# jilljenn/TF-recomm

Measured on AMD Instinct MI355X. Metric: training ratings/sec + val RMSE, MovieLens-1M SVD dim=64 @1 GPU, higher is better.
Workload: dtype f32

## Files before the change

tf-recomm_amd/csrc/svd_kernels.hip:

```cpp
#include <hip/hip_runtime.h>
#include <stdint.h>
#include "svd_kernels.h"
#include "forward_body.h"
#include "finalize.inc.h"

namespace tfr {

template <int VEC>
__device__ __forceinline__ void store_frag(float* __restrict__ row, int d0, int D, const Frag<VEC>& f) {
    if (d0 < D) {
        if constexpr (VEC == 4) {
            *reinterpret_cast<float4*>(row + d0) = make_float4(f.v[0], f.v[1], f.v[2], f.v[3]);
        } else {
            row[d0] = f.v[0];
        }
    }
}

template <int VEC, bool NT>
__device__ __forceinline__ Frag<VEC> load_full(const float* __restrict__ p) {
    Frag<VEC> f;
    if constexpr (VEC == 4) {
        floatx4 t;
        if constexpr (NT) t = __builtin_nontemporal_load(reinterpret_cast<const floatx4*>(p));
        else t = *reinterpret_cast<const floatx4*>(p);
        f.v[0] = t.x; f.v[1] = t.y; f.v[2] = t.z; f.v[3] = t.w;
    } else {
        if constexpr (NT) f.v[0] = __builtin_nontemporal_load(p);
        else f.v[0] = *p;
    }
    return f;
}

template <int VEC>
__device__ __forceinline__ Frag<VEC> load_frag_h(const float* __restrict__ row, int d0, int D, bool nt) {
    return nt ? load_frag<VEC, true>(row, d0, D) : load_frag<VEC, false>(row, d0, D);
}
template <int VEC>
__device__ __forceinline__ void store_frag_h(float* __restrict__ row, int d0, int D, const Frag<VEC>& f, bool nt) {
    if (!nt) { store_frag<VEC>(row, d0, D, f); return; }
    if (d0 < D) {
        if constexpr (VEC == 4) {
            floatx4 t; t.x = f.v[0]; t.y = f.v[1]; t.z = f.v[2]; t.w = f.v[3];
            __builtin_nontemporal_store(t, reinterpret_cast<floatx4*>(row + d0));
        } else {
            __builtin_nontemporal_store(f.v[0], row + d0);
        }
    }
}

__device__ __forceinline__ __amdgpu_buffer_rsrc_t wt_rsrc(const void* base) {
    return __builtin_amdgcn_make_buffer_rsrc(const_cast<void*>(base), 0, 0x7fffffff, 0x00020000);
}
template <int VEC>
__device__ __forceinline__ void store_frag_wt(__amdgpu_buffer_rsrc_t r, size_t off, int d0, int D, const Frag<VEC>& f) {
    if (d0 < D) {
        if constexpr (VEC == 4) {
            typedef unsigned uintx4 __attribute__((ext_vector_type(4)));
            uintx4 t;
            t.x = __float_as_uint(f.v[0]); t.y = __float_as_uint(f.v[1]); t.z = __float_as_uint(f.v[2]); t.w = __float_as_uint(f.v[3]);
            __builtin_amdgcn_raw_buffer_store_b128(t, r, (int)((off + d0) * 4), 0, 16);
        } else {
            __builtin_amdgcn_raw_buffer_store_b32(__float_as_uint(f.v[0]), r, (int)((off + d0) * 4), 0, 16);
        }
    }
}
template <int VEC>
__device__ __forceinline__ void store_frag_p(float* base, size_t off, int d0, int D, const Frag<VEC>& f, bool wt) {
    if (wt) store_frag_wt<VEC>(wt_rsrc(base), off, d0, D, f);
    else store_frag<VEC>(base + off, d0, D, f);
}
__device__ __forceinline__ void store_word_p(void* base, size_t idx, uint32_t x, bool wt) {
    if (wt) __builtin_amdgcn_raw_buffer_store_b32(x, wt_rsrc(base), (int)(idx * 4), 0, 16);
    else reinterpret_cast<uint32_t*>(base)[idx] = x;
}

constexpr int BUF_NONE = (int)0x80000000u;
__device__ __forceinline__ uint32_t buf_load_word(__amdgpu_buffer_rsrc_t r, int byte_off) {
    return __builtin_amdgcn_raw_buffer_load_b32(r, byte_off, 0, 0);
}
template <int VEC>
__device__ __forceinline__ Frag<VEC> buf_load_frag(__amdgpu_buffer_rsrc_t r, int byte_off) {
    Frag<VEC> f;
    if constexpr (VEC == 4) {
        typedef unsigned uintx4 __attribute__((ext_vector_type(4)));
        const uintx4 t = __builtin_amdgcn_raw_buffer_load_b128(r, byte_off, 0, 0);
        f.v[0] = __uint_as_float(t.x); f.v[1] = __uint_as_float(t.y); f.v[2] = __uint_as_float(t.z); f.v[3] = __uint_as_float(t.w);
    } else {
        f.v[0] = __uint_as_float(buf_load_word(r, byte_off));
    }
    return f;
}

template <int G, int EPG>
__device__ __forceinline__ void block_sum_pieces(const float (&val)[3 * EPG], float* stage, float* out) {
    constexpr int EPB = 1024 / G;
    const int tid = threadIdx.x, lane = tid & 63, wave = tid >> 6;
    const int grp = tid / G, gl = tid % G;
    float* sl = stage;
    float* sg = stage + EPG * EPB;
    float* sr = stage + 2 * EPG * EPB;
#pragma unroll
    for (int h = 0; h < EPG; ++h) {
        if (gl == 0) { sl[h * EPB + grp] = val[3 * h + 0]; sg[h * EPB + grp] = val[3 * h + 2]; }
        sr[h * 1024 + tid] = val[3 * h + 1];
    }
    __syncthreads();
    if (wave < 3 * EPG) {
        const int h = wave / 3, c = wave % 3;
        float x = 0.f;
        if (c == 1) {
#pragma unroll
            for (int k = 0; k < 16; ++k) x += sr[h * 1024 + k * 64 + lane];
        } else {
            const float* src = (c == 0 ? sl : sg) + h * EPB;
            for (int k = lane; k < EPB; k += 64) x += src[k];
        }
        x = wave_sum(x);
        if (lane == 0) out[h * 4 + c] = x;
    }
}

template <int G, int VEC, int MODE, int UNR, bool PNT>
__global__ __launch_bounds__(256) void k_forward(FwdArgs a) {
    warm_args(a);
    forward_body<Float32Rows<VEC>, G, MODE, UNR, 4, PNT>(a, blockIdx.x, gridDim.x);
}
__device__ __forceinline__ void tile_scan_pack(int32_t* cnt, int nb, int32_t* wtot) {
    const int tid = threadIdx.x, lane = tid & 63, wave = tid >> 6;
    const int per = (nb + 1023) / 1024;
    int32_t sum = 0;
    for (int q = 0; q < per; ++q) { const int b = q * 1024 + tid; if (b < nb) sum += cnt[b]; }
    int32_t incl = sum;
#pragma unroll
    for (int o = 1; o < 64; o <<= 1) {
        const int32_t t2 = __shfl_up(incl, o, 64);
        if (lane >= o) incl += t2;
    }
    if (lane == 63) wtot[wave] = incl;
    __syncthreads();
    int32_t run = incl - sum;
    for (int w = 0; w < wave; ++w) run += wtot[w];
    for (int q = 0; q < per; ++q) {
        const int b = q * 1024 + tid;
        if (b < nb) { const int32_t c2 = cnt[b]; cnt[b] = (c2 << 16) | run; run += c2; }
    }
    __syncthreads();
}

template <int G, int VEC>
__global__ __launch_bounds__(1024) void k_front(FrontArgs fa) {
    warm_args(fa);
    if ((int)blockIdx.x < fa.nfwd) {
        forward_body<Float32Rows<VEC>, G, MODE_TRAIN, 2, 16>(fa.f, blockIdx.x, fa.nfwd);
        return;
    }
    extern __shared__ int32_t cnt[];
    const CSortArgs& a = fa.c;
    const int rb = blockIdx.x - fa.nfwd;
    const int col = rb / a.ntiles, tile = rb % a.ntiles, tid = threadIdx.x;
    const int nb = a.nbins[col];
    for (int b = tid; b < nb; b += CSORT_TILE) cnt[b] = 0;
    __syncthreads();
    const int64_t k = (int64_t)tile * CSORT_TILE + tid;
    const bool valid = k < a.B;
    int32_t key = 0, fullkey = 0;
    if (valid) {
        if (fa.f.ids) {
            int64_t id = fa.f.ids[k];
            if ((uint64_t)id >= (uint64_t)fa.f.N) id = 0;
            const int4 rec = fa.f.store[id];
            fullkey = col == 0 ? rec.x : rec.y;
            fa.key_out[col][k] = fullkey;
        } else {
            fullkey = a.keys[col][k];
        }
        key = fullkey & (nb - 1);
    }
    unsigned long long mask = __ballot(valid);
    for (int bit = 1; bit < nb; bit <<= 1) {
        const unsigned long long m = __ballot((key & bit) != 0);
        mask &= (key & bit) ? m : ~m;
    }
    const int lane = tid & 63, wave = tid >> 6;
    const unsigned long long below = mask & ((1ull << lane) - 1ull);
    const int rank_in_wave = __popcll(below);
    const int group_size = __popcll(mask);
    int base = 0;
    for (int w = 0; w < CSORT_TILE / 64; ++w) {
        if (wave == w && valid) {
            base = cnt[key];
            if (below == 0) cnt[key] = base + group_size;
        }
        __syncthreads();
    }
    if (!fa.tile_local) {
        if (valid) a.lrank[col][k] = base + rank_in_wave;
        for (int b = tid; b < nb; b += CSORT_TILE) a.hist[col][(size_t)tile * nb + b] = cnt[b];
        return;
    }
    __shared__ int32_t wtot[256];
    tile_scan_pack(cnt, nb, wtot);
    for (int b = tid; b < nb; b += CSORT_TILE) a.hist[col][(size_t)tile * nb + b] = cnt[b];
    if (valid) {
        const int64_t dst = (int64_t)tile * CSORT_TILE + (cnt[key] & 0xffff) + base + rank_in_wave;
        a.ks[col][dst] = fullkey;
        a.ps[col][dst] = (int32_t)k;
    }
}

struct TileLds {
    int32_t* cnt; int32_t* rec_u; int32_t* rec_i; float* rec_r; int32_t* srt_key; int32_t* srt_pos; int32_t* wtot;
};
__device__ __forceinline__ void tile_sort(int32_t* cnt_, int32_t* rec_u_, int32_t* rec_i_, float* rec_r_, int32_t* srt_key_,
                                          int32_t* srt_pos_, int32_t* wtot_, const int64_t* ids, const int4* store, const int4* recs,
                                          const int32_t* bu_, const int32_t* bi_, const float* br_, int64_t tile0, int nvalid, int side,
                                          int nb, int64_t N, int64_t U, int64_t I, int32_t* err, bool have_rec, int4 rec_in) {
    TileLds L;
    L.cnt = cnt_; L.rec_u = rec_u_; L.rec_i = rec_i_; L.rec_r = rec_r_; L.srt_key = srt_key_; L.srt_pos = srt_pos_; L.wtot = wtot_;
    const int tid = threadIdx.x, lane = tid & 63, wave = tid >> 6;
    for (int b = tid; b < nb; b += 1024) L.cnt[b] = 0;
    const bool valid = tid < nvalid;
    int32_t u = 0, it = 0;
    float r = 0.f;
    if (valid) {
        const int64_t k = tile0 + tid;
        bool oob = false;
        if (have_rec) {
            u = rec_in.x; it = rec_in.y; r = __int_as_float(rec_in.z);
        } else if (recs) {
            const int4 rec = recs[k];
            u = rec.x; it = rec.y; r = __int_as_float(rec.z);
        } else if (ids) {
            int64_t id = ids[k];
            if ((uint64_t)id >= (uint64_t)N) { atomicOr(err, 2); id = 0; }
            const int4 rec = store[id];
            u = rec.x; it = rec.y; r = __int_as_float(rec.z);
        } else {
            u = bu_[k]; it = bi_[k]; r = br_[k];
        }
        if ((uint64_t)(int64_t)u >= (uint64_t)U) { oob = true; u = 0; }
        if ((uint64_t)(int64_t)it >= (uint64_t)I) { oob = true; it = 0; }
        if (oob) atomicOr(err, 1);
    }
    L.rec_u[tid] = u; L.rec_i[tid] = it; L.rec_r[tid] = r;
    __syncthreads();
    const int32_t key = side == 0 ? u : it;
    unsigned long long mask = __ballot(valid);
    for (int bit = 1; bit < nb; bit <<= 1) {
        const unsigned long long mm = __ballot((key & bit) != 0);
        mask &= (key & bit) ? mm : ~mm;
    }
    const unsigned long long below = mask & ((1ull << lane) - 1ull);
    const int rank_in_wave = __popcll(below);
    const int group_size = __popcll(mask);
    int base = 0;
    for (int w = 0; w < 16; ++w) {
        if (wave == w && valid) {
            base = L.cnt[key];
            if (below == 0) L.cnt[key] = base + group_size;
        }
        __syncthreads();
    }
    tile_scan_pack(L.cnt, nb, L.wtot);
    if (valid) {
        const int dst = (L.cnt[key] & 0xffff) + base + rank_in_wave;
        L.srt_key[dst] = key;
        L.srt_pos[dst] = tid;
    }
    __syncthreads();
}

__device__ __forceinline__ void zero_tail(float* partials, int from, int to) {
    if (from < to) for (int k = from + (int)threadIdx.x; k < to; k += 1024) partials[k] = 0.f;
}

struct TileStamp {
    unsigned long long* p; unsigned long long t0;
    __device__ __forceinline__ void arm(unsigned long long* dbg) { p = dbg ? dbg + 8 * (size_t)blockIdx.x : nullptr; }
    __device__ __forceinline__ void mark(int k) const { if (p && threadIdx.x == 0) p[k] = __builtin_amdgcn_s_memrealtime(); }
    __device__ __forceinline__ ~TileStamp() { if (p && threadIdx.x == 0) { p[0] = t0; p[1] = __builtin_amdgcn_s_memrealtime(); } }
};

template <int G, int VEC, int EPG, bool PRE>
__device__ __forceinline__ void tile_pieces(const TileStepArgs& a, int32_t* dyn, const int32_t* rec_u, const int32_t* rec_i,
                                            const float* rec_r, const int32_t* srt_key, const int32_t* srt_pos, float* lds_gb,
                                            int32_t* lds_key, float* lds_stage, TileStamp& stamp, int side, int bx, int slice,
                                            int64_t tile0, int nvalid, const int4* srt, const WarmLines<TileStepArgs>& warm,
                                            int zero_from, int zero_to);

template <int G, int VEC, int EPG>
__global__ __launch_bounds__(1024) void k_tile_step(const int4* srt_u, const int4* srt_i, const int4* next_recs, int B, int nsort, int nblk_u,
                                                    int epg_item, int ntiles, int next_ntiles, int next_B, int stamps, TileStepArgs a) {
    const WarmLines<TileStepArgs> warm = warm_args_issue(a);
    constexpr int EPB = 1024 / G;
    extern __shared__ __attribute__((aligned(16))) int32_t dyn[];
    __shared__ int32_t rec_u[1024], rec_i[1024], srt_key[1024], srt_pos[1024];
    __shared__ float rec_r[1024];
    __shared__ __attribute__((aligned(16))) float lds_gb[2 * EPG * 16];
    __shared__ __attribute__((aligned(16))) int32_t lds_key[EPG * 16];
    __shared__ float lds_stage[EPG * (2 * EPB + 1024)];
    __shared__ int32_t wtot[16];
    static_assert(sizeof(rec_u) + sizeof(rec_i) + sizeof(srt_key) + sizeof(srt_pos) + sizeof(rec_r) + sizeof(lds_gb) + sizeof(lds_key) +
                  sizeof(lds_stage) + sizeof(wtot) == tile_step_static_lds(G, EPG), "tile_step_static_lds() is out of date");
    static_assert(tile_step_static_lds(G, EPG) + 64 * 1024 <= LDS_PER_CU, "static LDS leaves no room for 16384 sort bins");
    TileStamp stamp = {nullptr, stamps ? __builtin_amdgcn_s_memrealtime() : 0ull};
    const int tid = threadIdx.x;
    const bool ahead = (int)blockIdx.x < nsort;
    const int b0 = (int)blockIdx.x - nsort;
    const int side = ahead ? (int)blockIdx.x / next_ntiles : (b0 < nblk_u ? 0 : 1);
    const int bx = ahead ? 0 : (side ? b0 - nblk_u : b0);
    const int epg = side ? epg_item : EPG;
    const int EPS = EPB * epg;
    const int NSL = 1024 / EPS;
    const int tile = ahead ? (int)blockIdx.x % next_ntiles : bx / NSL;
    const int slice = bx % NSL;
    const int64_t tile0 = (int64_t)tile * 1024;
    const int Bt = ahead ? next_B : B;
    const int nvalid = (Bt - (int)tile0 < 1024) ? Bt - (int)tile0 : 1024;
    const int zero_from = (!ahead && side == 1 && (int64_t)(bx + 1) * EPS >= B) ? (bx + 1) * epg * 4 : INT32_MAX;
    const int zero_to = ntiles * G * 4;
    if (!ahead && slice * EPS >= nvalid) {
        stamp.arm(a.dbg);
        zero_tail(a.partials, zero_from, zero_to);
        if (side == 1 && tid < 4 * epg) a.partials[(size_t)bx * epg * 4 + tid] = 0.f;
        return;
    }
    if (!ahead && srt_u != nullptr) {
        const int4* srt = side ? srt_i : srt_u;
        if constexpr (EPG > 1) {
            if (epg != EPG) {
                tile_pieces<G, VEC, EPG / 2, true>(a, dyn, rec_u, rec_i, rec_r, srt_key, srt_pos, lds_gb, lds_key, lds_stage, stamp, side, bx,
                                                   slice, tile0, nvalid, srt, warm, zero_from, zero_to);
                return;
            }
        }
        tile_pieces<G, VEC, EPG, true>(a, dyn, rec_u, rec_i, rec_r, srt_key, srt_pos, lds_gb, lds_key, lds_stage, stamp, side, bx, slice,
                                       tile0, nvalid, srt, warm, zero_from, zero_to);
        return;
    }
    {
        const bool early = ahead && next_recs != nullptr;
        int4 early_rec = make_int4(0, 0, 0, 0);
        if (early) early_rec = next_recs[tile0 + (tid < nvalid ? tid : 0)];
        __builtin_amdgcn_sched_barrier(0);
        warm_args_land(warm);
        stamp.arm(a.dbg);
        zero_tail(a.partials, zero_from, zero_to);
        const int nb = a.nbins[side];
        tile_sort(dyn, rec_u, rec_i, rec_r, srt_key, srt_pos, wtot, ahead ? a.next_ids : a.ids, a.store, ahead ? next_recs : a.recs,
                  a.u, a.it, a.r, tile0, nvalid, side, nb, a.N, a.U, a.I, a.err, early, early_rec);
        const bool wt = a.wt & TFR_WT_PUBLISH;
        if (ahead) {
            int32_t* nt = a.next_tab[side];
            for (int b = tid; b < nb; b += 1024) store_word_p(nt, (size_t)tile * nb + b, (uint32_t)dyn[b], wt);
            if (tid < nvalid) {
                const int pl = srt_pos[tid];
                const int4 rec = make_int4(rec_u[pl], rec_i[pl], __float_as_int(rec_r[pl]), pl);
                if (wt) {
                    typedef unsigned uintx4 __attribute__((ext_vector_type(4)));
                    uintx4 t; t.x = (unsigned)rec.x; t.y = (unsigned)rec.y; t.z = (unsigned)rec.z; t.w = (unsigned)rec.w;
                    __builtin_amdgcn_raw_buffer_store_b128(t, wt_rsrc(a.next_srt[side]), (int)((tile0 + tid) * 16), 0, 16);
                } else {
                    a.next_srt[side][tile0 + tid] = rec;
                }
            }
            return;
        }
        const int nact = (nvalid + EPS - 1) / EPS;
        for (int b = slice * 1024 + tid; b < nb; b += nact * 1024) store_word_p(a.tab[side], (size_t)tile * nb + b, (uint32_t)dyn[b], wt);
        __syncthreads();
    }
    if constexpr (EPG > 1) {
        if (epg != EPG) {
            tile_pieces<G, VEC, EPG / 2, false>(a, dyn, rec_u, rec_i, rec_r, srt_key, srt_pos, lds_gb, lds_key, lds_stage, stamp, side, bx, slice,
                                                tile0, nvalid, nullptr, warm, zero_from, zero_to);
            return;
        }
    }
    tile_pieces<G, VEC, EPG, false>(a, dyn, rec_u, rec_i, rec_r, srt_key, srt_pos, lds_gb, lds_key, lds_stage, stamp, side, bx, slice, tile0,
                                    nvalid, nullptr, warm, zero_from, zero_to);
}

template <int G, int VEC, int EPG, bool PRE>
__device__ __forceinline__ void tile_pieces(const TileStepArgs& a, int32_t* dyn, const int32_t* rec_u, const int32_t* rec_i,
                                            const float* rec_r, const int32_t* srt_key, const int32_t* srt_pos, float* lds_gb,
                                            int32_t* lds_key, float* lds_stage, TileStamp& stamp, int side, int bx, int slice,
                                            int64_t tile0, int nvalid, const int4* srt, const WarmLines<TileStepArgs>& warm,
                                            int zero_from, int zero_to) {
    constexpr bool presorted = PRE;
    constexpr int EPB = 1024 / G;
    constexpr int EPS = EPB * EPG;
    const int tid = threadIdx.x;
    const int grp = tid / G, gl = tid % G, d0 = gl * VEC;
    int jl[EPG], bpos[EPG];
// ... 569 lines not shown
        if (gl == 0) {
            a.grad_bias[j] = gb;
            if (head && a.map) a.map[row] = (int32_t)j + 1;
        }
    } else if constexpr (RMODE == RMODE_ADAM) {
        if (!a.frozen_rows) {
            Frag<VEC> w;
            if constexpr (OWN_LDS) w = wre;
            else w = (FWD && LEAN) ? load_frag<VEC>(wsrc, d0, D) : o;
#pragma unroll
            for (int q = 0; q < VEC; ++q) adam_sparse(w.v[q], mrow.v[q], vrow.v[q], acc.v[q], c);
            const bool nts = FAST || (a.nt & 4);
            store_frag_h<VEC>(wdst, d0, D, w, nts);
            if (a.sel && gl == 0) a.sel[row] = cur ^ 1;
            store_frag_h<VEC>(a.m + roff, d0, D, mrow, nts);
            store_frag_h<VEC>(a.v + roff, d0, D, vrow, nts);
        }
        if (gl == 0 && !a.frozen_bias) {
            float w = ob;
            adam_sparse(w, mb, vb, gb, c);
            a.bias_w[row] = w;
            a.bias_m[row] = mb;
            a.bias_v[row] = vb;
        }
    } else if constexpr (RMODE == RMODE_SGD) {
        if (!a.frozen_rows) {
            Frag<VEC> w = o;
#pragma unroll
            for (int q = 0; q < VEC; ++q) w.v[q] = w.v[q] - a.lr * acc.v[q];
            store_frag<VEC>(wdst, d0, D, w);
            if (a.sel && gl == 0) a.sel[row] = cur ^ 1;
        }
        if (gl == 0 && !a.frozen_bias) a.bias_w[row] = ob - a.lr * gb;
    }
}

template <int VEC, int N>
__device__ __forceinline__ bool add_pieces(Frag<VEC>& t, float& gb, const float* __restrict__ grad_rows,
                                           const float* __restrict__ grad_bias, const int32_t* __restrict__ ks,
                                           int64_t B, int64_t safe, int64_t p, int64_t step, int32_t row, int d0, int D) {
    int32_t key[N];
#pragma unroll
    for (int q = 0; q < N; ++q) {
        const int64_t pp = p + (int64_t)q * step;
        key[q] = ks[pp < B ? pp : safe];
    }
    Frag<VEC> x[N];
    float xb[N];
#pragma unroll
    for (int q = 0; q < N; ++q) {
        const int64_t pp = (p + (int64_t)q * step < B) ? p + (int64_t)q * step : safe;
        x[q] = load_frag<VEC>(grad_rows + (size_t)pp * D, d0, D);
        xb[q] = grad_bias[pp];
    }
    bool go = true;
#pragma unroll
    for (int q = 0; q < N; ++q) {
        go = go && (p + (int64_t)q * step < B) && key[q] == row;
        if (go) {
#pragma unroll
            for (int e = 0; e < VEC; ++e) t.v[e] += x[q].v[e];
            gb += xb[q];
        }
    }
    return go;
}

template <int VEC, int PIECE>
__device__ __forceinline__ Frag<VEC> run_total(const float* __restrict__ grad_rows,
                                               const float* __restrict__ grad_bias,
                                               const int32_t* __restrict__ ks, int64_t B, int64_t j,
                                               int32_t row, int d0, int D, float& gb) {
    Frag<VEC> t = load_frag<VEC>(grad_rows + (size_t)j * D, d0, D);
    gb = grad_bias[j];
    int64_t p = (j / PIECE + 1) * PIECE;
    if (p >= B || ks[p] != row) return t;
    while (add_pieces<VEC, 8>(t, gb, grad_rows, grad_bias, ks, B, j, p, PIECE, row, d0, D)) p += 8 * (int64_t)PIECE;
    return t;
}

template <int G, int VEC, int OPT>
__global__ __launch_bounds__(256) void k_apply_rows(ApplyPair pr) {
    warm_args(pr.a[blockIdx.y]);
    constexpr int PIECE = 1024 / G;
    constexpr int GPB = 256 / G;
    constexpr int CW = 16;
    if (pr.with_fin && blockIdx.x == gridDim.x - 1) {
        if (blockIdx.y == 0) finalize_body(pr.f);
        return;
    }
    __shared__ float s_part[256 * VEC];
    __shared__ float s_partb[GPB];
    __shared__ long long s_next[GPB];
    __shared__ int32_t s_row[GPB];
    const ApplyArgs& a = pr.a[blockIdx.y];
    const int32_t err = *a.err;
    const int gl = threadIdx.x % G, grp = threadIdx.x / G;
    const int d0 = gl * VEC;
    const int D = a.D;
    const int64_t Bn = a.dB ? (int64_t)*a.dB : a.B;
    int64_t j = (int64_t)blockIdx.x * GPB + grp;
    int32_t row = 0;
    bool own;
    if (a.only_split) {
        const int64_t p = (j + 1) * PIECE;
        own = !err && p < Bn;
        if (own) {
            row = a.ks[p];
            const int64_t lo = p - PIECE;
            own = a.ks[p - 1] == row && !(lo > 0 && a.ks[lo - 1] == row);
            if (own) {
                const int sh = ((threadIdx.x % 64) / G) * G;
                j = p - 1;
                for (int k = 0; k < PIECE; k += G) {
                    const bool hit = (k + gl < PIECE) && a.ks[lo + k + gl] == row;
                    unsigned long long bits = __ballot(hit) >> sh;
                    if constexpr (G < 64) bits &= (1ull << G) - 1ull;
                    if (bits) { j = lo + k + (__ffsll((long long)bits) - 1); break; }
                }
            }
        }
    } else {
        own = !err && j < Bn;
        if (own) {
            row = a.ks[j];
            own = ((j > 0) ? a.ks[j - 1] : -2) != row;
        }
    }
    const size_t roff = (size_t)row * D;
    Frag<VEC> w, mrow, vrow, gr;
#pragma unroll
    for (int q = 0; q < VEC; ++q) { w.v[q] = 0.f; mrow.v[q] = 0.f; vrow.v[q] = 0.f; gr.v[q] = 0.f; }
    float gb = 0.f;
    long long next = -1;
    float* wtab = a.w;
    if (own) {
        if (a.sel && a.sel[row]) wtab = a.w_alt;
        if (OPT != 2 && !a.frozen_rows) {
            w = load_frag<VEC>(wtab + roff, d0, D);
            if constexpr (OPT == 0) {
                mrow = load_frag<VEC>(a.m + roff, d0, D);
                vrow = load_frag<VEC>(a.v + roff, d0, D);
            }
        }
        gr = load_frag<VEC>(a.grad_rows + (size_t)j * D, d0, D);
        gb = a.grad_bias[j];
        const int64_t p = (j / PIECE + 1) * PIECE;
        if (p < Bn && a.ks[p] == row &&
            add_pieces<VEC, 8>(gr, gb, a.grad_rows, a.grad_bias, a.ks, Bn, j, p, PIECE, row, d0, D))
            next = p + 8 * (int64_t)PIECE;
    }
    if (gl == 0) { s_next[grp] = next; s_row[grp] = row; }
    if (__syncthreads_or(next >= 0)) {
        for (int sl = 0; sl < GPB; ++sl) {
            const long long ps = s_next[sl];
            if (ps < 0) continue;
            const int32_t rs = s_row[sl];
            Frag<VEC> part;
#pragma unroll
            for (int q = 0; q < VEC; ++q) part.v[q] = 0.f;
            float pb = 0.f;
            int64_t pp = ps + (int64_t)grp * PIECE;
            while (add_pieces<VEC, CW>(part, pb, a.grad_rows, a.grad_bias, a.ks, Bn, 0, pp, (int64_t)GPB * PIECE, rs, d0, D))
                pp += (int64_t)CW * GPB * PIECE;
#pragma unroll
            for (int q = 0; q < VEC; ++q) s_part[threadIdx.x * VEC + q] = part.v[q];
            if (gl == 0) s_partb[grp] = pb;
            __syncthreads();
            if (grp == sl) {
                for (int g2 = 0; g2 < GPB; ++g2) {
#pragma unroll
                    for (int q = 0; q < VEC; ++q) gr.v[q] += s_part[(g2 * G + gl) * VEC + q];
                    gb += s_partb[g2];
                }
            }
            __syncthreads();
        }
    }
    if (!own) return;
    const AdamC c = {a.alpha, a.b1, a.b2, a.eps, 1.f - a.b1, 1.f - a.b2};
    if constexpr (OPT == 2) {
        store_frag<VEC>(a.w + (a.wstride ? (size_t)row * a.wstride : roff), d0, D, gr);
        if (gl == 0) a.bias_w[a.wbstride ? (size_t)row * a.wbstride : (size_t)row] = gb;
        return;
    }
    if (!a.frozen_rows) {
        if constexpr (OPT == 0) {
#pragma unroll
            for (int q = 0; q < VEC; ++q) adam_sparse(w.v[q], mrow.v[q], vrow.v[q], gr.v[q], c);
            store_frag<VEC>(a.m + roff, d0, D, mrow);
            store_frag<VEC>(a.v + roff, d0, D, vrow);
        } else {
#pragma unroll
            for (int q = 0; q < VEC; ++q) w.v[q] = w.v[q] - a.lr * gr.v[q];
        }
        store_frag<VEC>(wtab + roff, d0, D, w);
    }
    if (gl == 0 && !a.frozen_bias) {
        float bw = a.bias_w[row];
        if constexpr (OPT == 0) {
            float mb = a.bias_m[row], vb = a.bias_v[row];
            adam_sparse(bw, mb, vb, gb, c);
            a.bias_m[row] = mb;
            a.bias_v[row] = vb;
        } else {
            bw = bw - a.lr * gb;
        }
        a.bias_w[row] = bw;
    }
}

template <int G, int VEC>
__global__ __launch_bounds__(256) void k_adam_dense(DensePair pr) {
    constexpr int PIECE = 1024 / G;
    if (blockIdx.y == 2) {
        if (blockIdx.x == 0) finalize_body(pr.f);
        return;
    }
    warm_args(pr.a[blockIdx.y]);
    const DenseArgs& a = pr.a[blockIdx.y];
    if (*a.err) return;
    constexpr int GPB = 256 / G;
    const int gl = threadIdx.x % G;
    const int d0 = gl * VEC;
    const int D = a.D;
    const AdamC c = {a.alpha, a.b1, a.b2, a.eps, 1.f - a.b1, 1.f - a.b2};
    for (int64_t row = (int64_t)blockIdx.x * GPB + threadIdx.x / G; row < a.rows;
         row += (int64_t)gridDim.x * GPB) {
        const int32_t slot = a.map ? a.map[row] : 0;
        const size_t roff = (size_t)row * D;
        Frag<VEC> w, mrow, vrow;
#pragma unroll
        for (int q = 0; q < VEC; ++q) { w.v[q] = 0.f; mrow.v[q] = 0.f; vrow.v[q] = 0.f; }
        if (!a.frozen_rows) {
            w = load_frag<VEC>(a.w + roff, d0, D);
            if (a.opt == 0) {
                mrow = load_frag<VEC>(a.m + roff, d0, D);
                vrow = load_frag<VEC>(a.v + roff, d0, D);
            }
        }
        float bw = 0.f, mb = 0.f, vb = 0.f;
        if (gl == 0 && !a.frozen_bias) {
            bw = a.bias_w[row];
            if (a.opt == 0) { mb = a.bias_m[row]; vb = a.bias_v[row]; }
        }
        Frag<VEC> gr;
        float gb = 0.f;
        if (a.dense_grad) {
            gr = load_frag<VEC>(a.dense_grad + roff, d0, D);
            gb = a.dense_gbias[row];
            if (slot) {
                gr = run_total<VEC, PIECE>(a.grad_rows, a.grad_bias, a.ks, a.B, (int64_t)slot - 1, (int32_t)row, d0, D, gb);
                if (gl == 0) a.map[row] = 0;
            }
            Frag<VEC> z;
#pragma unroll
            for (int q = 0; q < VEC; ++q) z.v[q] = 0.f;
            store_frag<VEC>(a.dense_grad + roff, d0, D, z);
            if (gl == 0) a.dense_gbias[row] = 0.f;
        } else if (slot) {
            gr = run_total<VEC, PIECE>(a.grad_rows, a.grad_bias, a.ks, a.B, (int64_t)slot - 1, (int32_t)row, d0, D, gb);
            if (gl == 0) a.map[row] = 0;
        } else {
#pragma unroll
            for (int q = 0; q < VEC; ++q) gr.v[q] = 0.f;
        }
        if (!a.frozen_rows) {
            if (a.opt == 0) {
#pragma unroll
                for (int q = 0; q < VEC; ++q) adam_sparse(w.v[q], mrow.v[q], vrow.v[q], gr.v[q], c);
                store_frag<VEC>(a.m + roff, d0, D, mrow);
                store_frag<VEC>(a.v + roff, d0, D, vrow);
            } else {
#pragma unroll
                for (int q = 0; q < VEC; ++q) w.v[q] = w.v[q] - a.lr * gr.v[q];
            }
            store_frag<VEC>(a.w + roff, d0, D, w);
        }
        if (gl == 0 && !a.frozen_bias) {
            if (a.opt == 0) {
                adam_sparse(bw, mb, vb, gb, c);
                a.bias_m[row] = mb;
                a.bias_v[row] = vb;
            } else {
                bw = bw - a.lr * gb;
            }
            a.bias_w[row] = bw;
        }
    }
}

struct DenseHead { const int32_t* tab; const int32_t* err; int nbins, rows, ntiles; };
template <int G, int VEC, bool WRITE, int NT>
__device__ __forceinline__ void dense_tiles_rounds(const TileDenseLaunch& L, const DenseHead& h, const WarmLines<TileDenseArgs>& warm) {
    const TileDenseArgs& a = L.a[blockIdx.y];
    constexpr int GPB = 256 / G;
    constexpr int EPB = 1024 / G;
    constexpr int D = G * VEC;
    constexpr int NB = (NT > 12) ? 8 : NT;
    const int gl = threadIdx.x % G;
    const int d0 = gl * VEC;
    const int row = (int)blockIdx.x * GPB + threadIdx.x / G;
    if (row >= h.rows) return;
    const __amdgpu_buffer_rsrc_t rtab =
        __builtin_amdgcn_make_buffer_rsrc(const_cast<int32_t*>(h.tab), 0, h.ntiles * h.nbins * 4, 0x00020000);
    int32_t ent[NT];
#pragma unroll
    for (int t = 0; t < NT; ++t) ent[t] = (int32_t)buf_load_word(rtab, (t * h.nbins + row) * 4);
    int32_t err = (int32_t)buf_load_word(wt_rsrc(h.err), 0);
    __builtin_amdgcn_sched_barrier(0);
    warm_args_land(warm);
    const int roff = (row * D + d0) * 4;
    Frag<VEC> w, mrow, vrow;
    float bw = 0.f, mb = 0.f, vb = 0.f;
    if constexpr (!WRITE) {
        const int ow = a.frozen_rows ? BUF_NONE : roff;
        const int om = (a.frozen_rows || a.opt != 0) ? BUF_NONE : roff;
        w = buf_load_frag<VEC>(wt_rsrc(a.w), ow);
        mrow = buf_load_frag<VEC>(wt_rsrc(a.m), om);
        vrow = buf_load_frag<VEC>(wt_rsrc(a.v), om);
        const int ob = (gl == 0 && !a.frozen_bias) ? row * 4 : BUF_NONE;
        const int obm = (gl == 0 && !a.frozen_bias && a.opt == 0) ? row * 4 : BUF_NONE;
        bw = __uint_as_float(buf_load_word(wt_rsrc(a.bias_w), ob));
        mb = __uint_as_float(buf_load_word(wt_rsrc(a.bias_m), obm));
        vb = __uint_as_float(buf_load_word(wt_rsrc(a.bias_v), obm));
    }
    __builtin_amdgcn_sched_barrier(0);
    asm volatile("" : "+v"(err) : : "memory");
    if (err) return;
    int s0 = -1, s1 = -1, nk1 = 0;
    bool deep = false, touched = false;
#pragma unroll
    for (int t = 0; t < NT; ++t) {
        const int32_t e = ent[t];
        const int off = e & 0xffff;
        const int pp = t * 1024 + (off / EPB + 1) * EPB;
        const int end = t * 1024 + off + (e >> 16);
        const bool has1 = pp < end;
        deep = deep || pp + EPB < end;
        s1 = (has1 && nk1 == 1) ? pp : s1;
        s0 = (has1 && nk1 == 0) ? pp : s0;
        nk1 += has1 ? 1 : 0;
        touched = touched || (e >> 16);
    }
    const __amdgpu_buffer_rsrc_t rg = wt_rsrc(a.grad_rows), rgb = wt_rsrc(a.grad_bias);
    Frag<VEC> tot, c0, c1;
#pragma unroll
    for (int q = 0; q < VEC; ++q) tot.v[q] = 0.f;
    float gb = 0.f, cb0 = 0.f, cb1 = 0.f;
#pragma unroll
    for (int t0 = 0; t0 < NT; t0 += NB) {
        Frag<VEC> x[NB];
        float xb[NB];
#pragma unroll
        for (int t = 0; t < NB; ++t) {
            const int32_t e = ent[t0 + t];
            const int j = (t0 + t) * 1024 + (e & 0xffff);
            x[t] = buf_load_frag<VEC>(rg, (e >> 16) ? (j * D + d0) * 4 : BUF_NONE);
            xb[t] = __uint_as_float(buf_load_word(rgb, ((e >> 16) && gl == 0) ? j * 4 : BUF_NONE));
        }
        if (t0 == 0) {
            c0 = buf_load_frag<VEC>(rg, s0 >= 0 ? (s0 * D + d0) * 4 : BUF_NONE);
            cb0 = __uint_as_float(buf_load_word(rgb, (s0 >= 0 && gl == 0) ? s0 * 4 : BUF_NONE));
            c1 = buf_load_frag<VEC>(rg, s1 >= 0 ? (s1 * D + d0) * 4 : BUF_NONE);
            cb1 = __uint_as_float(buf_load_word(rgb, (s1 >= 0 && gl == 0) ? s1 * 4 : BUF_NONE));
        }
        __builtin_amdgcn_sched_barrier(0);
#pragma unroll
        for (int t = 0; t < NB; ++t) {
#pragma unroll
            for (int q = 0; q < VEC; ++q) tot.v[q] += x[t].v[q];
            gb += xb[t];
        }
    }
    if (nk1 <= 2 && !deep) {
#pragma unroll
        for (int q = 0; q < VEC; ++q) tot.v[q] += c0.v[q];
        gb += cb0;
#pragma unroll
        for (int q = 0; q < VEC; ++q) tot.v[q] += c1.v[q];
        gb += cb1;
    } else {
        for (int k = 1;; ++k) {
            bool more = false;
#pragma unroll
            for (int t0 = 0; t0 < NT; t0 += NB) {
                Frag<VEC> y[NB];
                float yb[NB];
#pragma unroll
                for (int t = 0; t < NB; ++t) {
                    const int32_t e = ent[t0 + t];
                    const int j = (t0 + t) * 1024 + (e & 0xffff);
                    const int pp = (j / EPB + k) * EPB;
                    const bool has = pp < j + (e >> 16);
                    y[t] = buf_load_frag<VEC>(rg, has ? (pp * D + d0) * 4 : BUF_NONE);
                    yb[t] = __uint_as_float(buf_load_word(rgb, (has && gl == 0) ? pp * 4 : BUF_NONE));
                    more = more || has;
                }
#pragma unroll
                for (int t = 0; t < NB; ++t) {
#pragma unroll
                    for (int q = 0; q < VEC; ++q) tot.v[q] += y[t].v[q];
                    gb += yb[t];
                }
            }
            if (!more) break;
        }
    }
    const size_t rfl = (size_t)row * D;
    if constexpr (WRITE) {
        if (touched) {
            store_frag<VEC>(a.out_rows + rfl, d0, D, tot);
            if (gl == 0) a.out_bias[row] = gb;
        }
    } else {
        if (!touched && a.skip_untouched) return;
        const AdamC c = {a.alpha, a.b1, a.b2, a.eps, 1.f - a.b1, 1.f - a.b2};
        const int wt = L.wt;
        if (!a.frozen_rows) {
            if (a.opt == 0) {
#pragma unroll
                for (int q = 0; q < VEC; ++q) adam_sparse(w.v[q], mrow.v[q], vrow.v[q], tot.v[q], c);
                store_frag_p<VEC>(a.m, rfl, d0, D, mrow, wt & TFR_WT_MOMENTS);
                store_frag_p<VEC>(a.v, rfl, d0, D, vrow, wt & TFR_WT_MOMENTS);
            } else {
#pragma unroll
                for (int q = 0; q < VEC; ++q) w.v[q] = __builtin_fmaf(-a.lr, tot.v[q], w.v[q]);
            }
            store_frag_p<VEC>(a.w, rfl, d0, D, w, wt & TFR_WT_ROWS);
        }
        if (gl == 0 && !a.frozen_bias) {
            const bool wb = wt & TFR_WT_BIAS;
            if (a.opt == 0) {
                adam_sparse(bw, mb, vb, gb, c);
                store_word_p(a.bias_m, (size_t)row, __float_as_uint(mb), wb);
                store_word_p(a.bias_v, (size_t)row, __float_as_uint(vb), wb);
            } else {
                bw = bw - __fmul_rn(a.lr, gb);
            }
            store_word_p(a.bias_w, (size_t)row, __float_as_uint(bw), wb);
        }
    }
}

template <int G, int VEC, bool WRITE, int NT>
__global__ __launch_bounds__(256, (NT > 12 && VEC == 4 && !WRITE) ? 2 : 3)
void k_dense_tiles(const int32_t* tab0, const int32_t* tab1, const int32_t* errp, int nbins0, int nbins1, int rows0, int rows1, int ntiles,
                   int ncols, int flags, TileDenseLaunch L) {
    const WarmLines<TileDenseArgs> warm = warm_args_issue(L.a[blockIdx.y]);
    if ((int)blockIdx.x == ncols) {
        if (blockIdx.y == 0 && (flags & DENSE_FLAG_FIN)) finalize_body(L.f);
        return;
    }
    const bool users = blockIdx.y != 0;
    const DenseHead h = {users ? tab1 : tab0, errp, users ? nbins1 : nbins0, users ? rows1 : rows0, ntiles};
    if constexpr (VEC == 4) {
        if (flags & DENSE_FLAG_ROUNDS) {
            dense_tiles_rounds<G, VEC, WRITE, NT>(L, h, warm);
            return;
        }
    }
    const TileDenseArgs& a = L.a[blockIdx.y];
    const int32_t err = *h.err;
    warm_args_land(warm);
    constexpr int GPB = 256 / G;
    constexpr int EPB = 1024 / G;
    const int gl = threadIdx.x % G;
    const int d0 = gl * VEC;
    const int D = a.D;
    const AdamC c = {a.alpha, a.b1, a.b2, a.eps, 1.f - a.b1, 1.f - a.b2};
    for (int64_t row = (int64_t)blockIdx.x * GPB + threadIdx.x / G; row < h.rows;
         row += (int64_t)ncols * GPB) {
        const size_t roff = (size_t)row * D;
        Frag<VEC> w, mrow, vrow;
#pragma unroll
        for (int q = 0; q < VEC; ++q) { w.v[q] = 0.f; mrow.v[q] = 0.f; vrow.v[q] = 0.f; }
        float bw = 0.f, mb = 0.f, vb = 0.f;
        if constexpr (!WRITE) {
            if (!a.frozen_rows) {
                w = load_frag<VEC>(a.w + roff, d0, D);
                if (a.opt == 0) {
                    mrow = load_frag<VEC>(a.m + roff, d0, D);
                    vrow = load_frag<VEC>(a.v + roff, d0, D);
                }
            }
            if (gl == 0 && !a.frozen_bias) {
                bw = a.bias_w[row];
                if (a.opt == 0) { mb = a.bias_m[row]; vb = a.bias_v[row]; }
            }
        }
        Frag<VEC> tot;
#pragma unroll
        for (int q = 0; q < VEC; ++q) tot.v[q] = 0.f;
        float gb = 0.f;
        bool touched = false;
        constexpr int NB = (NT > 12) ? 8 : NT;
        int32_t ent[NT];
#pragma unroll
        for (int t = 0; t < NT; ++t) ent[t] = (t < h.ntiles) ? h.tab[(size_t)t * h.nbins + row] : 0;
        if (err) return;
#pragma unroll
        for (int t0 = 0; t0 < NT; t0 += NB) {
            Frag<VEC> x[NB];
            float xb[NB];
#pragma unroll
            for (int t = 0; t < NB; ++t) {
                const int32_t e = ent[t0 + t];
#pragma unroll
                for (int q = 0; q < VEC; ++q) x[t].v[q] = 0.f;
                xb[t] = 0.f;
                if (e >> 16) {
                    const int64_t j = (int64_t)(t0 + t) * 1024 + (e & 0xffff);
                    x[t] = load_frag<VEC>(a.grad_rows + (size_t)j * D, d0, D);
                    xb[t] = a.grad_bias[j];
                }
            }
#pragma unroll
            for (int t = 0; t < NB; ++t) {
                if (ent[t0 + t] >> 16) {
                    touched = true;
#pragma unroll
                    for (int q = 0; q < VEC; ++q) tot.v[q] += x[t].v[q];
                    gb += xb[t];
                }
            }
        }
        for (int k = 1;; ++k) {
            bool more = false;
#pragma unroll
            for (int t0 = 0; t0 < NT; t0 += NB) {
                Frag<VEC> y[NB];
                float yb[NB];
#pragma unroll
                for (int t = 0; t < NB; ++t) {
                    const int32_t e = ent[t0 + t];
                    const int64_t j = (int64_t)(t0 + t) * 1024 + (e & 0xffff);
                    const int64_t pp = (j / EPB + k) * EPB;
                    const bool has = (e >> 16) && pp < j + (e >> 16);
#pragma unroll
                    for (int q = 0; q < VEC; ++q) y[t].v[q] = 0.f;
                    yb[t] = 0.f;
                    if (has) {
                        y[t] = load_frag<VEC>(a.grad_rows + (size_t)pp * D, d0, D);
                        yb[t] = a.grad_bias[pp];
                        more = true;
                    }
                }
#pragma unroll
                for (int t = 0; t < NB; ++t) {
#pragma unroll
                    for (int q = 0; q < VEC; ++q) tot.v[q] += y[t].v[q];
                    gb += yb[t];
                }
            }
            if (!more) break;
        }
        if constexpr (WRITE) {
            if (touched) {
                store_frag<VEC>(a.out_rows + roff, d0, D, tot);
                if (gl == 0) a.out_bias[row] = gb;
            }
        } else {
            if (!touched && a.skip_untouched) continue;
            const int wt = L.wt;
            if (!a.frozen_rows) {
                if (a.opt == 0) {
#pragma unroll
                    for (int q = 0; q < VEC; ++q) adam_sparse(w.v[q], mrow.v[q], vrow.v[q], tot.v[q], c);
                    store_frag_p<VEC>(a.m, roff, d0, D, mrow, wt & TFR_WT_MOMENTS);
                    store_frag_p<VEC>(a.v, roff, d0, D, vrow, wt & TFR_WT_MOMENTS);
                } else {
#pragma unroll
                    for (int q = 0; q < VEC; ++q) w.v[q] = w.v[q] - a.lr * tot.v[q];
                }
                store_frag_p<VEC>(a.w, roff, d0, D, w, wt & TFR_WT_ROWS);
            }
            if (gl == 0 && !a.frozen_bias) {
                const bool wb = wt & TFR_WT_BIAS;
                if (a.opt == 0) {
                    adam_sparse(bw, mb, vb, gb, c);
                    store_word_p(a.bias_m, (size_t)row, __float_as_uint(mb), wb);
                    store_word_p(a.bias_v, (size_t)row, __float_as_uint(vb), wb);
                } else {
                    bw = bw - a.lr * gb;
                }
                store_word_p(a.bias_w, (size_t)row, __float_as_uint(bw), wb);
            }
        }
    }
}

__global__ __launch_bounds__(256) void k_finalize(FinArgs a) { warm_args(a); finalize_body(a); }

__global__ __launch_bounds__(256) void k_auc_keys(const float* __restrict__ score, int32_t* __restrict__ keys, int64_t n) {
    for (int64_t k = (int64_t)blockIdx.x * blockDim.x + threadIdx.x; k < n; k += (int64_t)gridDim.x * blockDim.x) {
        float x = score[k];
        if (x == 0.f) x = 0.f;
        const uint32_t b = __float_as_uint(x);
        keys[k] = (int32_t)((b & 0x80000000u) ? ~b : (b | 0x80000000u));
    }
}

__global__ __launch_bounds__(256) void k_auc_ranksum(const int32_t* __restrict__ ks, const int32_t* __restrict__ ps,
                                                     const float* __restrict__ label, int64_t n, unsigned long long* out ) {
    unsigned long long s2 = 0, np = 0;
    for (int64_t j = (int64_t)blockIdx.x * blockDim.x + threadIdx.x; j < n; j += (int64_t)gridDim.x * blockDim.x) {
        if (label[ps[j]] > 0.5f) {
            const uint32_t key = (uint32_t)ks[j];
            int64_t lo = 0, hi = n;
            while (lo < hi) { const int64_t mid = (lo + hi) >> 1; if ((uint32_t)ks[mid] < key) lo = mid + 1; else hi = mid; }
            const int64_t first = lo;
            hi = n;
            while (lo < hi) { const int64_t mid = (lo + hi) >> 1; if ((uint32_t)ks[mid] <= key) lo = mid + 1; else hi = mid; }
            s2 += (unsigned long long)(first + lo + 1);
            np += 1;
        }
    }
    for (int o = 32; o >= 1; o >>= 1) { s2 += __shfl_down(s2, o, 64); np += __shfl_down(np, o, 64); }
    if ((threadIdx.x & 63) == 0 && np) { atomicAdd(&out[0], s2); atomicAdd(&out[1], np); }
}

void launch_auc_keys(const float* score, int32_t* keys, int64_t n, hipStream_t s) {
    hipLaunchKernelGGL(k_auc_keys, dim3(blocks_for(n, 256, 2048)), dim3(256), 0, s, score, keys, n);
}
void launch_auc_ranksum(const int32_t* ks, const int32_t* ps, const float* label, int64_t n, unsigned long long* out, hipStream_t s) {
    hipLaunchKernelGGL(k_auc_ranksum, dim3(blocks_for(n, 256, 2048)), dim3(256), 0, s, ks, ps, label, n, out);
}

__device__ __forceinline__ uint64_t splitmix64(uint64_t x) {
    x += 0x9E3779B97F4A7C15ull;
    x = (x ^ (x >> 30)) * 0xBF58476D1CE4E5B9ull;
    x = (x ^ (x >> 27)) * 0x94D049BB133111EBull;
    return x ^ (x >> 31);
}

__global__ __launch_bounds__(256) void k_init_trunc_normal(float* p, int64_t n, float stddev, uint64_t seed) {
    for (int64_t k = (int64_t)blockIdx.x * blockDim.x + threadIdx.x; k < n;
         k += (int64_t)gridDim.x * blockDim.x) {
        float z = 0.f;
        for (int attempt = 0; attempt < 16; ++attempt) {
            const uint64_t h = splitmix64(seed ^ splitmix64((uint64_t)k * 16 + attempt));
            const float u1 = ((float)(uint32_t)(h >> 40) + 0.5f) * (1.f / 16777216.f);
            const float u2 = ((float)(uint32_t)((h >> 16) & 0xFFFFFF) + 0.5f) * (1.f / 16777216.f);
            z = sqrtf(-2.f * __logf(u1)) * __cosf(6.28318530718f * u2);
            if (fabsf(z) <= 2.f) break;
            z = 0.f;
        }
        p[k] = z * stddev;
    }
}

__global__ void k_init_uniform_scalar(float* p, float lo, float hi, uint64_t seed) {
    const uint64_t h = splitmix64(seed ^ 0xABCDEF12345ull);
    const float u = ((float)(uint32_t)(h >> 40) + 0.5f) * (1.f / 16777216.f);
    p[0] = lo + (hi - lo) * u;
}

template <int MODE, int UNR>
static void launch_forward_mode(const FwdArgs& a, int G, int VEC, int grid, hipStream_t s) {
    with_geometry(G, VEC, [&](auto g, auto v) {
        with_bool(forward_pnt(MODE, a.U, a.D), [&](auto pnt) {
            hipLaunchKernelGGL((k_forward<g.value, v.value, MODE, UNR, pnt.value>), dim3(grid), dim3(256), 0, s, a);
        });
    });
}

int forward_grid(int64_t B, int G, int mode, int unr) {
    return blocks_for(B, 4 * (64 / G) * unr, (mode == MODE_INFER) ? 8192 : 2048);
}

int front_forward_blocks(int64_t B, int G) {
    return blocks_for(B, 16 * (64 / G) * 2, 512);
}

void launch_front(const FrontArgs& fa, int G, int VEC, hipStream_t s) {
    const int nbmax = fa.c.nbins[0] > fa.c.nbins[1] ? fa.c.nbins[0] : fa.c.nbins[1];
    const dim3 grid(fa.nfwd + 2 * fa.c.ntiles);
    with_geometry(G, VEC, [&](auto g, auto v) {
        static bool attr = false;
        if (!attr) {
            (void)hipFuncSetAttribute(reinterpret_cast<const void*>(k_front<g.value, v.value>),
                                      hipFuncAttributeMaxDynamicSharedMemorySize, CSORT_MAX_BINS * 4);
            attr = true;
        }
        hipLaunchKernelGGL((k_front<g.value, v.value>), grid, dim3(1024), (size_t)nbmax * 4, s, fa);
    });
}

int tile_step_epg(int ntiles, int G, int VEC) {
    auto fits = [&](int e) {
        return (size_t)2 * e * 16 * G * VEC * 4 <= (size_t)64 * 1024 && tile_step_static_lds(G, e) + (size_t)64 * 1024 <= LDS_PER_CU;
    };
    static const int forced = (int)env_int("TFR_EPG", 0);
    if (forced == 1 || ((forced == 2 || forced == 4) && forced <= G && fits(forced))) return forced;
    int epg = 1;
    while (epg < 4 && epg < G && ntiles * (G / epg) * 2 > 256 && fits(2 * epg)) epg *= 2;
    return epg;
}

int tile_step_item_epg(int64_t B, int G, int VEC, int nsort) {
    const int epg = tile_step_epg((int)((B + 1023) / 1024), G, VEC);
    static const bool split = env_default_off("TFR_ITEM_SPLIT");
    if (!split || epg < 2) return epg;
    const int64_t epb = 1024 / G;
    const int64_t nu = (B + epb * epg - 1) / (epb * epg), ni = (B + epb * (epg / 2) - 1) / (epb * (epg / 2));
    return nsort + nu + ni <= 256 ? epg / 2 : epg;
}
int tile_step_one_barrier() {
    static const bool on = env_default_off("TFR_ONE_BARRIER");
    return on;
}
int tile_step_wt() {
    static_assert((TFR_WT_DEFAULT & 31) == TFR_WT_DEFAULT, "five bits");
    static const int wt = (int)env_int("TFR_WT", TFR_WT_DEFAULT) & 31;
    return wt;
}

void launch_tile_step(const TileStepArgs& a0, int G, int VEC, hipStream_t s) {
    const int nbmax = a0.nbins[0] > a0.nbins[1] ? a0.nbins[0] : a0.nbins[1];
    const int epg = tile_step_epg(a0.ntiles, G, VEC);
    size_t dyn = (size_t)nbmax * 4;
    if (dyn < (size_t)2 * epg * 16 * G * VEC * 4) dyn = (size_t)2 * epg * 16 * G * VEC * 4;
    if (tile_step_static_lds(G, epg) + dyn > LDS_PER_CU) return;
    const int nsort = a0.next_ids ? 2 * a0.next_ntiles : 0;
    TileStepArgs a = a0;
    a.epg_item = tile_step_item_epg(a.B, G, VEC, nsort);
    a.one_barrier = tile_step_one_barrier();
    a.wt = tile_step_wt();
    const int64_t epb = 1024 / G;
    const int nblk_u = (int)((a.B + epb * epg - 1) / (epb * epg)), nblk_i = (int)((a.B + epb * a.epg_item - 1) / (epb * a.epg_item));
    const dim3 grid(nsort + nblk_u + nblk_i);
    with_geometry(G, VEC, [&](auto g, auto v) {
        with_one_of<1, 2, 4>(epg, [&](auto e) {
// ... 162 lines not shown
```

Baseline: 630.3 million.

## Spread tile-table and bias loads across group lanes and broadcast via DPP

Instead of every lane in a row group loading all NT tile-table entries, each lane loads a strided subset and the values are broadcast within the group using DPP row broadcasts or shuffles. Per-tile grad-bias loads are likewise distributed across lanes and broadcast, and the three bias/moment words are fetched by different lanes (selected by gl%3) with pointer selection, then broadcast. This cuts redundant per-lane memory instructions and VGPR pressure in the dense tile reduction. In exchange it adds cross-lane broadcast operations and relies on the group fitting within DPP row constraints (G of 4 or at least 16), falling back to shuffles otherwise.

```diff
diff --git a/tf-recomm_amd/csrc/svd_kernels.hip b/tf-recomm_amd/csrc/svd_kernels.hip
--- a/tf-recomm_amd/csrc/svd_kernels.hip
+++ b/tf-recomm_amd/csrc/svd_kernels.hip
@@ -1,5 +1,6 @@
 #include <hip/hip_runtime.h>
 #include <stdint.h>
+#include <utility>
 #include "svd_kernels.h"
 #include "forward_body.h"
 #include "finalize.inc.h"
@@ -91,6 +92,18 @@
     }
     return f;
 }
+
+template <int G, int L>
+__device__ __forceinline__ uint32_t group_bcast(uint32_t x) {
+    static_assert(L < G && L < 16, "group_bcast: L is a lane of the group's 16-lane row");
+    if constexpr (G >= 16) return (uint32_t)__builtin_amdgcn_update_dpp(0, (int)x, 0x150 + L, 0xf, 0xf, false);
+    else if constexpr (G == 4) return (uint32_t)__builtin_amdgcn_update_dpp(0, (int)x, L * 0x55, 0xf, 0xf, false);
+    else return (uint32_t)__shfl((int)x, L, G);
+}
+template <int... K, typename F>
+__device__ __forceinline__ void unrolled(std::integer_sequence<int, K...>, F&& f) { (f(std::integral_constant<int, K>{}), ...); }
+template <int N, typename F>
+__device__ __forceinline__ void unrolled(F&& f) { unrolled(std::make_integer_sequence<int, N>{}, f); }
 
 template <int G, int EPG>
 __device__ __forceinline__ void block_sum_pieces(const float (&val)[3 * EPG], float* stage, float* out) {
@@ -1266,32 +1279,45 @@
     const int d0 = gl * VEC;
     const int row = (int)blockIdx.x * GPB + threadIdx.x / G;
     if (row >= h.rows) return;
+    constexpr int GE = G < 16 ? G : 16;
+    constexpr int NE = (NT + GE - 1) / GE;
+    constexpr int NS = (NT + 2 + GE - 1) / GE;
+    const int tl = gl % GE;
+    const bool first_row = G <= 16 || gl < 16;
     const __amdgpu_buffer_rsrc_t rtab =
         __builtin_amdgcn_make_buffer_rsrc(const_cast<int32_t*>(h.tab), 0, h.ntiles * h.nbins * 4, 0x00020000);
-    int32_t ent[NT];
-#pragma unroll
-    for (int t = 0; t < NT; ++t) ent[t] = (int32_t)buf_load_word(rtab, (t * h.nbins + row) * 4);
+    int32_t own[NS];
+#pragma unroll
+    for (int i = 0; i < NS; ++i) own[i] = i < NE ? (int32_t)buf_load_word(rtab, ((i * GE + tl) * h.nbins + row) * 4) : 0;
     int32_t err = (int32_t)buf_load_word(wt_rsrc(h.err), 0);
     __builtin_amdgcn_sched_barrier(0);
     warm_args_land(warm);
     const int roff = (row * D + d0) * 4;
     Frag<VEC> w, mrow, vrow;
-    float bw = 0.f, mb = 0.f, vb = 0.f;
+    uint32_t b3 = 0;
     if constexpr (!WRITE) {
         const int ow = a.frozen_rows ? BUF_NONE : roff;
         const int om = (a.frozen_rows || a.opt != 0) ? BUF_NONE : roff;
         w = buf_load_frag<VEC>(wt_rsrc(a.w), ow);
         mrow = buf_load_frag<VEC>(wt_rsrc(a.m), om);
         vrow = buf_load_frag<VEC>(wt_rsrc(a.v), om);
-        const int ob = (gl == 0 && !a.frozen_bias) ? row * 4 : BUF_NONE;
-        const int obm = (gl == 0 && !a.frozen_bias && a.opt == 0) ? row * 4 : BUF_NONE;
-        bw = __uint_as_float(buf_load_word(wt_rsrc(a.bias_w), ob));
-        mb = __uint_as_float(buf_load_word(wt_rsrc(a.bias_m), obm));
-        vb = __uint_as_float(buf_load_word(wt_rsrc(a.bias_v), obm));
+        const bool mom = (a.opt == 0) & !a.frozen_bias;
+        uint64_t pw = (uint64_t)a.bias_w, pm = (uint64_t)a.bias_m, pv = (uint64_t)a.bias_v;
+        asm volatile("" : "+s"(pw), "+s"(pm), "+s"(pv));
+        uint64_t bp = pw;
+        bp = (mom & (gl % 3 == 1)) ? pm : bp;
+        bp = (mom & (gl % 3 == 2)) ? pv : bp;
+        typedef const float __attribute__((address_space(1))) gfloat;
+        b3 = __float_as_uint(reinterpret_cast<gfloat*>(bp)[row]);
     }
     __builtin_amdgcn_sched_barrier(0);
     asm volatile("" : "+v"(err) : : "memory");
     if (err) return;
+    int32_t ent[NT];
+    unrolled<NT>([&](auto tc) {
+        constexpr int t = decltype(tc)::value;
+        ent[t] = (int32_t)group_bcast<G, t % GE>((uint32_t)own[t / GE]);
+    });
     int s0 = -1, s1 = -1, nk1 = 0;
     bool deep = false, touched = false;
 #pragma unroll
@@ -1311,46 +1337,63 @@
     Frag<VEC> tot, c0, c1;
 #pragma unroll
     for (int q = 0; q < VEC; ++q) tot.v[q] = 0.f;
-    float gb = 0.f, cb0 = 0.f, cb1 = 0.f;
+    float gb = 0.f;
+    uint32_t sb[NS];
 #pragma unroll
     for (int t0 = 0; t0 < NT; t0 += NB) {
         Frag<VEC> x[NB];
-        float xb[NB];
+        if (t0 == 0) {
+#pragma unroll
+            for (int i = 0; i < NS; ++i) {
+                const int slot = i * GE + tl;
+                const int32_t e = own[i];
+                int at = (e >> 16) ? slot * 1024 + (e & 0xffff) : -1;
+                at = slot == NT ? s0 : slot == NT + 1 ? s1 : at;
+                sb[i] = buf_load_word(rgb, (at >= 0 && first_row) ? at * 4 : BUF_NONE);
+            }
+        }
 #pragma unroll
         for (int t = 0; t < NB; ++t) {
             const int32_t e = ent[t0 + t];
             const int j = (t0 + t) * 1024 + (e & 0xffff);
             x[t] = buf_load_frag<VEC>(rg, (e >> 16) ? (j * D + d0) * 4 : BUF_NONE);
-            xb[t] = __uint_as_float(buf_load_word(rgb, ((e >> 16) && gl == 0) ? j * 4 : BUF_NONE));
         }
         if (t0 == 0) {
             c0 = buf_load_frag<VEC>(rg, s0 >= 0 ? (s0 * D + d0) * 4 : BUF_NONE);
-            cb0 = __uint_as_float(buf_load_word(rgb, (s0 >= 0 && gl == 0) ? s0 * 4 : BUF_NONE));
             c1 = buf_load_frag<VEC>(rg, s1 >= 0 ? (s1 * D + d0) * 4 : BUF_NONE);
-            cb1 = __uint_as_float(buf_load_word(rgb, (s1 >= 0 && gl == 0) ? s1 * 4 : BUF_NONE));
         }
         __builtin_amdgcn_sched_barrier(0);
+        unrolled<NT>([&](auto tc) {
+            constexpr int t = decltype(tc)::value;
+            if (t >= t0 && t < t0 + NB) gb += __uint_as_float(group_bcast<G, t % GE>(sb[t / GE]));
+        });
 #pragma unroll
         for (int t = 0; t < NB; ++t) {
 #pragma unroll
             for (int q = 0; q < VEC; ++q) tot.v[q] += x[t].v[q];
-            gb += xb[t];
         }
     }
     if (nk1 <= 2 && !deep) {
 #pragma unroll
         for (int q = 0; q < VEC; ++q) tot.v[q] += c0.v[q];
-        gb += cb0;
+        gb += __uint_as_float(group_bcast<G, NT % GE>(sb[NT / GE]));
 #pragma unroll
         for (int q = 0; q < VEC; ++q) tot.v[q] += c1.v[q];
-        gb += cb1;
+        gb += __uint_as_float(group_bcast<G, (NT + 1) % GE>(sb[(NT + 1) / GE]));
     } else {
         for (int k = 1;; ++k) {
             bool more = false;
+            uint32_t yb[NE];
+#pragma unroll
+            for (int i = 0; i < NE; ++i) {
+                const int32_t e = own[i];
+                const int j = (i * GE + tl) * 1024 + (e & 0xffff);
+                const int pp = (j / EPB + k) * EPB;
+                yb[i] = buf_load_word(rgb, (pp < j + (e >> 16) && first_row) ? pp * 4 : BUF_NONE);
+            }
 #pragma unroll
             for (int t0 = 0; t0 < NT; t0 += NB) {
                 Frag<VEC> y[NB];
-                float yb[NB];
 #pragma unroll
                 for (int t = 0; t < NB; ++t) {
                     const int32_t e = ent[t0 + t];
@@ -1358,15 +1401,17 @@
                     const int pp = (j / EPB + k) * EPB;
                     const bool has = pp < j + (e >> 16);
                     y[t] = buf_load_frag<VEC>(rg, has ? (pp * D + d0) * 4 : BUF_NONE);
-                    yb[t] = __uint_as_float(buf_load_word(rgb, (has && gl == 0) ? pp * 4 : BUF_NONE));
                     more = more || has;
                 }
 #pragma unroll
                 for (int t = 0; t < NB; ++t) {
 #pragma unroll
                     for (int q = 0; q < VEC; ++q) tot.v[q] += y[t].v[q];
-                    gb += yb[t];
                 }
+                unrolled<NT>([&](auto tc) {
+                    constexpr int t = decltype(tc)::value;
+                    if (t >= t0 && t < t0 + NB) gb += __uint_as_float(group_bcast<G, t % GE>(yb[t / GE]));
+                });
             }
             if (!more) break;
         }
@@ -1393,6 +1438,8 @@
             }
             store_frag_p<VEC>(a.w, rfl, d0, D, w, wt & TFR_WT_ROWS);
         }
+        float bw = __uint_as_float(b3);
+        float mb = __uint_as_float(group_bcast<G, 1>(b3)), vb = __uint_as_float(group_bcast<G, 2>(b3));
         if (gl == 0 && !a.frozen_bias) {
             const bool wb = wt & TFR_WT_BIAS;
             if (a.opt == 0) {
```

Result: faster. 650.3 million, median of 6 (+3.2%).
